# icyveins7/pydsproutines

Hardware: AMD Instinct MI355X
Metric: CAF Msamples/s (4k template x 256 freq bins) (higher is better)
Workload: dtype f32

## Files before the change

### pydsproutines_amd/csrc/caf_fused.hip

```cpp
#include <algorithm>
#include <cstdlib>
#include <type_traits>

#include "caf_internal.h"
#include "caf_fft_dev.h"
#include "caf_wave.h"

namespace caf {

constexpr int FB = 16384;
constexpr int FP_P1 = 4384;
constexpr int FP_IM = 16 * FP_P1;
constexpr int F_LDS_BYTES = 2 * FP_IM;
constexpr int F_LDS_DATA = F_LDS_BYTES / 8;
__host__ __device__ constexpr int fp_row2(int n2) { return ((n2 >> 1) & 3) * 1088 + ((n2 & 1) + 2 * (n2 >> 3)) * 256; }
static_assert(fp_row2(15) + 256 <= FP_P1 && FP_P1 % 256 == 32, "planar image geometry");

#define CAF_AS1 __attribute__((address_space(1)))
#define CAF_AS4 __attribute__((address_space(4)))
typedef float v2f_t __attribute__((ext_vector_type(2)));
typedef float v4f_t __attribute__((ext_vector_type(4)));
typedef int v2i_t __attribute__((ext_vector_type(2)));
__device__ __forceinline__ float2 ld2(const float2* base, uint32_t elem) {
    const uint64_t u = *reinterpret_cast<const CAF_AS1 uint64_t*>((const CAF_AS1 char*)base + (elem << 3));
// ... 398 lines not shown
                bii = up ? pk_i[n4] : bii;
            }
            const uint32_t dloc = pk_d0 + (16u * bii + 64u * bq) * 64u;
            unsigned long long key = bvv < 0.f ? 0ull : (((unsigned long long)__float_as_uint(bvv) << 32) | (uint32_t)~dloc);
            key = wave_max(key);
            if ((tid & 63) == 0) {
                PeakRec r;
                r.v = key ? __uint_as_float((uint32_t)(key >> 32)) : -1.f;
                r.delay = key ? (int32_t)(f1->shift_start + f1_rel0 + (int64_t)(uint32_t)~(uint32_t)key) : 0x7fffffff;
                r.f = 0;
                f1->partial[(int64_t)h * f1->ppt + (int64_t)f1->blk_abs * 16 + (tid >> 6)] = r;
            }
        }
    }
    if (MODE == 2 || MODE == 5) {
        const int n1 = tid & 15, n2 = (tid >> 4) & 15, q = tid >> 8;
#pragma unroll
        for (int i = 0; i < 4; ++i)
#pragma unroll
            for (int n4 = 0; n4 < 4; ++n4) {
                const int tile = 16 * i + 64 * n4 + (n2 >> 2) + 4 * q;
                const int oo = 4 * i + n4;
                if (tile < tiles_per_blk) {
                    const uint32_t off = ((uint32_t)tile * 64u + (uint32_t)(n1 + 16 * (n2 & 3))) << 2;
                    gst1_wt(vt, off, bv[oo]);
                    __hip_atomic_store(reinterpret_cast<CAF_AS1 int32_t*>((CAF_AS1 char*)imax + off),
                                       (int32_t)(h0 + ((bi[oo >> 2] >> (8 * (oo & 3))) & 0xffu)), __ATOMIC_RELAXED,
                                       __HIP_MEMORY_SCOPE_AGENT);
                }
            }
    }
}

template <int N_> struct caf_ic { static constexpr int value = N_; };
template <int MODE, int NVH, bool FOLD, int R, bool PART = false>
__device__ __forceinline__ void fused_item2q(float2* __restrict__ s_d, const float2* __restrict__ s_tw2,
                                             const float2* __restrict__ s_tw3, const float2* __restrict__ xb,
                                             const float2* __restrict__ hc,
                                             const int32_t* __restrict__ shifts, const float2* __restrict__ tw1,
                                             int32_t table_mode, int32_t nfreq, int32_t nhyp, int blk, int h0, int h1,
                                             int32_t tiles_per_blk, float* __restrict__ vt, int32_t npart = 1,
                                             const F1Direct* __restrict__ f1 = nullptr) {
    static_assert(FOLD || R == 0, "the output residue exists in the folded form only");
    static_assert(MODE == 1 || MODE == 4, "|y|^2 tiles (write-through) or complex-QF rows");
    static_assert(!FOLD || NVH == 0, "folded form: only the lower half of each residue's transform holds valid delays");
    static_assert(!PART || FOLD, "partitioned templates ride on the folded form");
    constexpr int ROW = FOLD ? 4 * FB : 2 * FB;
    using pt_t = typename std::conditional<FOLD, float4, float2>::type;
    const int tid = threadIdx.x;
    const lds_char* img = (const lds_char*)s_d;
    const uint32_t img0 = __builtin_amdgcn_readfirstlane((uint32_t)(uintptr_t)img);
    const uint32_t wave_u = __builtin_amdgcn_readfirstlane((uint32_t)tid >> 6);
    const uint32_t m0_x1 = img0 + wave_u * 256u, m0_w = img0 + wave_u * (uint32_t)FP_P1;
    const uint32_t m2 = fp_m2((uint32_t)tid);
    const float2 w = ld2(tw1, 1024u + m2);
    float2 base0 = make_float2(1.f, 0.f);
    if (R) {
        float sn, cs;
        sincospif((float)m2 * (1.0f / 16384.0f), &sn, &cs);
        base0 = make_float2(cs, sn);
    }
    const float* xp = (const float*)(xb + (int64_t)blk * ROW);
    float* vt_blk = vt + (int64_t)blk * tiles_per_blk * nhyp * 64;
    const __amdgpu_buffer_rsrc_t rvt = buf_of(uniform_ptr(vt_blk), (uint32_t)tiles_per_blk * (uint32_t)nhyp * 256u);
    const int n1o = tid & 15, n2o = (tid >> 4) & 15, qo = tid >> 8;
    uint32_t f1_bytes = 0;
    int64_t f1_rel0 = 0;
    __amdgpu_buffer_rsrc_t rie = rvt, f1_r0 = rvt;
    float f1_ts = 0.f;
    if constexpr (MODE == 4) {
        f1_rel0 = (int64_t)f1->blk_abs * f1->step;
        int64_t nv = f1->num_shifts - f1_rel0;
        if (nv > f1->step) nv = f1->step;
        f1_bytes = (uint32_t)nv * 4u;
        rie = buf_of(uniform_ptr(f1->inv_e + f1_rel0), f1_bytes);
    }
    const float* hrow_o;
    uint32_t hb_o;
    const float* hrow_n;
    uint32_t hb_n;
    auto row_of = [&](int h, const float*& hrow, uint32_t& hb) {
        const int rows_per = PART ? npart : 1;
        if (table_mode) {
            hrow = (const float*)(hc + (int64_t)h * rows_per * ROW);
            hb = (uint32_t)tid;
        } else {
            const int t = h / nfreq;
            const int32_t sh = *((const CAF_AS4 int32_t*)shifts + (h - t * nfreq)) >> 1;
            hrow = (const float*)(hc + (int64_t)t * rows_per * ROW);
            hb = fp_hbase(m2, sh);
        }
    };
    auto issue = [&](pt_t* bx, pt_t* bh, const float* hrow, uint32_t hb, auto cc_, auto a0_, auto np_, uint32_t lz) __attribute__((always_inline)) {
        constexpr int CC = decltype(cc_)::value, A0 = decltype(a0_)::value, NP = decltype(np_)::value;
#pragma unroll
        for (int k = 0; k < NP; ++k) {
            const uint32_t a = (uint32_t)(A0 + k);
// ... 460 lines not shown
        float v = -1.f;
        if (lane < nrows) {
            v = s_rowv[lane];
            const int64_t o = (int64_t)t * num_shifts + rel0 + lane;
            if (row_max) row_max[o] = v < 0.f ? __builtin_nanf("") : v;
            if (row_arg) row_arg[o] = s_rowi[lane];
        }
        if (partial) {
            float b = v;
            int32_t bidx = lane;
            wave_argmax(b, bidx);
            if (lane == 0) {
                PeakRec r;
                r.v = b;
                r.delay = (int32_t)(shift_start + rel0 + bidx);
                r.f = s_rowi[bidx];
                partial[(int64_t)t * partial_per_tmpl + pidx] = r;
            }
        }
    }
}


constexpr int PQ_FFT_NEXT = 0, PQ_TR_NEXT = 1, PQ_FFT_XCD = 4, PQ_DONE = 12;
constexpr int PQ_TILES = 16;

__device__ __forceinline__ int32_t pq_load(const int32_t* p) {
    return __hip_atomic_load(p, __ATOMIC_RELAXED, __HIP_MEMORY_SCOPE_AGENT);
}
__device__ __forceinline__ const CAF_AS4 PersistParams* params_of(const PersistParams* p) {
    uint64_t v = reinterpret_cast<uint64_t>(p);
    asm volatile("" : "+s"(v));
    return reinterpret_cast<const CAF_AS4 PersistParams*>(v);
}
typedef float v4f_u_t __attribute__((ext_vector_type(4), aligned(4)));
typedef int v4i_u_t __attribute__((ext_vector_type(4), aligned(4)));

constexpr int TW_H = 32;
constexpr int TW_PITCH = TW_H + 1;
constexpr int TW_LDS = 64 * TW_PITCH;

template <bool SURF, int DS>
__device__ __forceinline__ void transpose_wave(float* __restrict__ lds, const PersistParams* pp, int z, int tile0) {
    const CAF_AS4 PersistParams* P = params_of(pp);
    const int32_t ntmpl = P->ntmpl, nfreq = P->nfreq, step = P->step, tiles_per_blk = P->tiles_per_blk;
    const int64_t num_shifts = P->num_shifts, shift_start = P->shift_start;
    const int wave_id = __builtin_amdgcn_readfirstlane((int)(threadIdx.x >> 6));
    const int lane = threadIdx.x & 63;
    float* s_w = lds + wave_id * TW_LDS;
    const int tile = tile0 + wave_id;
    if (tile >= tiles_per_blk) return;
    const int blk = P->blk0 + z;
    const int sl0 = DS == 2 ? 128 * (tile & 255) + (tile >> 8) : tile * 64;
    const int64_t rel0 = (int64_t)blk * step + sl0;
    int64_t nv = num_shifts - (int64_t)blk * step;
    if (nv > step) nv = step;
    const int nrows = sl0 < nv ? (int)min((int64_t)64, (nv - sl0 + DS - 1) / DS) : 0;
    const int64_t pidx = (int64_t)blk * tiles_per_blk + tile;
    PeakRec* partial = P->partial;
    const int64_t ppt = P->partial_per_tmpl;
    const int s4 = 4 * (lane & 15), fq = lane >> 4;
    const int nsteps = (nfreq + TW_H - 1) / TW_H;
    for (int t = 0; t < ntmpl; ++t) {
        if (nrows == 0) {
            if (lane == 0 && partial) {
                PeakRec r;
// ... 310 lines not shown
        if (wave_id == 0) {
            int32_t* pq = P->pq;
            const int n_fft = P->n_fft, n_tr = P->n_tr, ngroups = P->ngroups;
            int next = -1;
            const int t = __builtin_amdgcn_readfirstlane(pq_load(&pq[PQ_TR_NEXT]));
            if (t < n_tr) {
                const bool fft_left = __builtin_amdgcn_readfirstlane(pq_load(&pq[PQ_FFT_NEXT])) < n_fft;
                if (!fft_left || __builtin_amdgcn_readfirstlane(pq_load(&pq[PQ_DONE + t / ipb])) >= ngroups) {
                    int my = 0;
                    if (lane0) my = atomicAdd(&pq[PQ_TR_NEXT], 1);
                    my = __builtin_amdgcn_readfirstlane(my);
                    if (my < n_tr) {
                        pq_wait_block(pq, my, ipb, ngroups, lane0);
                        next = my;
                    }
                }
            }
            if (lane0) *s_next = next;
        }
        __syncthreads();
        item = __builtin_amdgcn_readfirstlane(*s_next);
        __syncthreads();
        if (item < 0) return;
    }
}

__device__ __forceinline__ void pq_mark(const PersistParams* pp, int slot, int v) {
    int32_t* d = params_of(pp)->dbg;
    if (d) __hip_atomic_store(&d[blockIdx.x * 8 + slot], v, __ATOMIC_RELAXED, __HIP_MEMORY_SCOPE_SYSTEM);
}

typedef __attribute__((address_space(3))) float2 lds_float2;
template <int KIND, int NV4>
__device__ __attribute__((noinline)) void persistent_fft_item(lds_float2* s_d, const lds_float2* s_tw2,
                                                              const lds_float2* s_tw3, const PersistParams* pp_in,
                                                              int item_in) {
    const PersistParams* pp = uniform_ptr(pp_in);
    const int item = __builtin_amdgcn_readfirstlane(item_in);
    const CAF_AS4 PersistParams* P = params_of(pp);
    const int ngroups = P->ngroups, hyp_per_wg = P->hyp_per_wg, nhyp = P->nhyp;
    const int blk = item / ngroups;
    const int grp = item - blk * ngroups;
    int h0 = grp * hyp_per_wg;
    int h1 = min(h0 + hyp_per_wg, nhyp);
    if (const int gpt = P->gpt) {
        const int t = grp / gpt;
        h0 = t * P->nfreq + (grp - t * gpt) * hyp_per_wg;
        h1 = min(h0 + hyp_per_wg, (t + 1) * P->nfreq);
    }
    if (KIND == 3) {
        F1Direct f1;
        f1.out0 = P->cqf;
        f1.out1 = nullptr;
        f1.partial = nullptr;
        f1.ppt = 0;
        f1.shift_start = 0;
        f1.inv_e = P->inv_e;
        f1.tscale = P->tscale;
        f1.num_shifts = P->num_shifts;
        f1.step = P->step;
        f1.blk_abs = P->blk0 + blk;
        fused_item<1024, 4, NV4>((float2*)s_d, (const float2*)s_tw2, (const float2*)s_tw3, P->xb, P->hc, P->shifts, P->tw1,
                                 P->table_mode, P->nfreq, nhyp, blk, h0, h1, P->tiles_per_blk, nullptr, nullptr, &f1);
    } else if (KIND == 2 || KIND == 4) {
        F1Direct f1;
        f1.out0 = P->row_max ? P->row_max : P->surface;
        f1.out1 = (P->row_max && P->surface) ? P->surface : nullptr;
        f1.inv_e = P->inv_e;
        f1.tscale = P->tscale;
        f1.num_shifts = P->num_shifts;
        f1.step = P->step;
        f1.blk_abs = P->blk0 + blk;
        f1.partial = P->partial;
        f1.ppt = P->partial_per_tmpl;
        f1.shift_start = P->shift_start;
        fused_item<1024, 3, NV4, KIND == 4>((float2*)s_d, (const float2*)s_tw2, (const float2*)s_tw3, P->xb, P->hc, P->shifts, P->tw1,
                                            P->table_mode, P->nfreq, nhyp, blk, h0, h1, P->tiles_per_blk, nullptr, nullptr, &f1);
    } else if (KIND == 5) {
        F1Direct f1;
        f1.out0 = P->surface_t;
        f1.out1 = nullptr;
        f1.partial = nullptr;
        f1.ppt = 0;
        f1.shift_start = 0;
        f1.inv_e = P->inv_e;
        f1.tscale = P->tscale;
        f1.num_shifts = P->num_shifts;
        f1.step = P->step;
        f1.blk_abs = P->blk0 + blk;
        const int64_t o = ((int64_t)blk * ngroups + grp) * P->tiles_per_blk * 64;
        fused_item<1024, 5, NV4>((float2*)s_d, (const float2*)s_tw2, (const float2*)s_tw3, P->xb, P->hc, P->shifts, P->tw1,
                                 P->table_mode, P->nfreq, nhyp, blk, h0, h1, P->tiles_per_blk, P->vmax + o, P->imax + o, &f1);
    } else if (KIND == 1) {
        const int64_t o = ((int64_t)blk * ngroups + grp) * P->tiles_per_blk * 64;
        fused_item<1024, 2, NV4>((float2*)s_d, (const float2*)s_tw2, (const float2*)s_tw3, P->xb, P->hc, P->shifts, P->tw1,
                            P->table_mode, P->nfreq, nhyp, blk, h0, h1, P->tiles_per_blk, P->vmax + o, P->imax + o);
    } else {
        fused_item<1024, 1, NV4>((float2*)s_d, (const float2*)s_tw2, (const float2*)s_tw3, P->xb, P->hc, P->shifts, P->tw1,
                            P->table_mode, P->nfreq, nhyp, blk, h0, h1, P->tiles_per_blk, P->vt);
    }
    __builtin_amdgcn_fence(__ATOMIC_RELEASE, "workgroup");
    __syncthreads();
    if (threadIdx.x == 0)
        __hip_atomic_fetch_add(&params_of(pp)->pq[PQ_DONE + blk], 1, __ATOMIC_RELAXED, __HIP_MEMORY_SCOPE_AGENT);
}

__device__ __forceinline__ void cq_params(const CAF_AS4 PersistParams* P, int blk, F1Direct& f1) {
    f1.out0 = P->cqf;
    f1.out1 = nullptr;
    f1.partial = nullptr;
    f1.ppt = 0;
    f1.shift_start = 0;
    f1.inv_e = P->inv_e;
    f1.tscale = P->tscale;
    f1.num_shifts = P->num_shifts;
    f1.step = P->step;
    f1.blk_abs = P->blk0 + blk;
}
template <int NVH, bool CQ>
__device__ __attribute__((noinline)) void persistent_fft_item2(lds_float2* s_d, const lds_float2* s_tw2, const lds_float2* s_tw3,
                                                               const PersistParams* pp_in, int item_in) {
    const PersistParams* pp = uniform_ptr(pp_in);
    const int item = __builtin_amdgcn_readfirstlane(item_in);
    const CAF_AS4 PersistParams* P = params_of(pp);
    const int ngroups = P->ngroups, hyp_per_wg = P->hyp_per_wg, nhyp = P->nhyp;
    const int blk = item / ngroups;
    const int grp = item - blk * ngroups;
    const int h0 = grp * hyp_per_wg;
    const int h1 = min(h0 + hyp_per_wg, nhyp);
    if constexpr (CQ) {
        F1Direct f1;
        cq_params(P, blk, f1);
        fused_item2q<4, NVH, false, 0>((float2*)s_d, (const float2*)s_tw2, (const float2*)s_tw3, P->xb, P->hc, P->shifts, P->tw1,
                                       P->table_mode, P->nfreq, nhyp, blk, h0, h1, P->tiles_per_blk, P->vt, 1, &f1);
    } else
    fused_item2q<1, NVH, false, 0>((float2*)s_d, (const float2*)s_tw2, (const float2*)s_tw3, P->xb, P->hc, P->shifts, P->tw1, P->table_mode,
                                   P->nfreq, nhyp, blk, h0, h1, P->tiles_per_blk, P->vt);
    __builtin_amdgcn_fence(__ATOMIC_RELEASE, "workgroup");
    __syncthreads();
    if (threadIdx.x == 0)
        __hip_atomic_fetch_add(&params_of(pp)->pq[PQ_DONE + blk], 1, __ATOMIC_RELAXED, __HIP_MEMORY_SCOPE_AGENT);
}

template <int R, bool PART, bool CQ>
__device__ __attribute__((noinline)) void persistent_fft_item2f(lds_float2* s_d, const lds_float2* s_tw2, const lds_float2* s_tw3,
                                                                const PersistParams* pp_in, int item_in) {
    const PersistParams* pp = uniform_ptr(pp_in);
    const int item = __builtin_amdgcn_readfirstlane(item_in);
    const CAF_AS4 PersistParams* P = params_of(pp);
    const int ngroups = P->ngroups, hyp_per_wg = P->hyp_per_wg, nhyp = P->nhyp;
    const int blk = item / ngroups;
    const int grp = (item - blk * ngroups) >> 1;
    const int h0 = grp * hyp_per_wg;
    const int h1 = min(h0 + hyp_per_wg, nhyp);
    if constexpr (CQ) {
        F1Direct f1;
        cq_params(P, blk, f1);
        fused_item2q<4, 0, true, R, PART>((float2*)s_d, (const float2*)s_tw2, (const float2*)s_tw3, P->xb, P->hc, P->shifts, P->tw1,
                                          P->table_mode, P->nfreq, nhyp, blk, h0, h1, P->tiles_per_blk, P->vt, PART ? P->npart : 1, &f1);
    } else
    fused_item2q<1, 0, true, R, PART>((float2*)s_d, (const float2*)s_tw2, (const float2*)s_tw3, P->xb, P->hc, P->shifts, P->tw1, P->table_mode,
                                      P->nfreq, nhyp, blk, h0, h1, P->tiles_per_blk, P->vt, PART ? P->npart : 1);
    __builtin_amdgcn_fence(__ATOMIC_RELEASE, "workgroup");
    __syncthreads();
    if (threadIdx.x == 0)
        __hip_atomic_fetch_add(&params_of(pp)->pq[PQ_DONE + blk], 1, __ATOMIC_RELAXED, __HIP_MEMORY_SCOPE_AGENT);
}

template <bool STATS>
__global__ __launch_bounds__(1024) void k_caf_persistent(const PersistParams* __restrict__ pp) {
    static_assert(16 * TW_LDS * 4 <= F_LDS_DATA * 8, "transposer patches must fit the FFT image");
    __shared__ __attribute__((aligned(16))) float2 s_d[F_LDS_DATA];
    __shared__ float2 s_tw2[2 * 16 * 64];
    __shared__ float2 s_tw3[2 * 16 * 4];
    __shared__ int32_t s_cmd[2];
    const int tid = threadIdx.x;
    {
        const CAF_AS4 PersistParams* P = params_of(pp);
        const float2* tw23 = P->tw23;
        s_tw2[tid] = tw23[tid];
        s_tw2[1024 + tid] = tw23[1088 + tid];
        if (tid < 64) {
            s_tw3[tid] = tw23[1024 + tid];
            s_tw3[64 + tid] = tw23[1088 + 1024 + tid];
        }
    }
    __syncthreads();
    const int wave_id = __builtin_amdgcn_readfirstlane(tid >> 6);
    const bool lane0 = (tid & 63) == 0;
    uint64_t tmark = STATS ? wall_clock64() : 0;
    const uint32_t t_start = (uint32_t)tmark;
    uint32_t t_claim = 0, t_fft = 0, t_tile = 0, c_fft = 0, c_tile = 0;
    for (;;) {
        if (wave_id == 0) {
            const CAF_AS4 PersistParams* P = params_of(pp);
            int32_t* pq = P->pq;
            const int n_fft = P->n_fft, n_tr = P->n_tr, ipb = P->ipb, ngroups = P->ngroups;
            const bool prefer_tr = (int)((blockIdx.x >> 3) & 31) >= 32 - P->tr_slots;
            int kind = 0, item = 0, spins = 0;
            for (;;) {
                const bool fft_left = __builtin_amdgcn_readfirstlane(pq_load(&pq[PQ_FFT_NEXT])) < n_fft;
                if (prefer_tr || !fft_left) {
                    const int t = __builtin_amdgcn_readfirstlane(pq_load(&pq[PQ_TR_NEXT]));
                    if (t < n_tr) {
                        if (!fft_left || __builtin_amdgcn_readfirstlane(pq_load(&pq[PQ_DONE + t / ipb])) >= ngroups) {
                            int my = 0;
                            if (lane0) my = atomicAdd(&pq[PQ_TR_NEXT], 1);
                            my = __builtin_amdgcn_readfirstlane(my);
                            if (my < n_tr) {
                                kind = 2;
                                item = my;
                                break;
                            }
                            continue;
                        }
                    } else if (!fft_left) {
                        break;
                    }
                }
                if (fft_left) {
                    const int nblk = P->nblk;
                    const int x0 = (int)(blockIdx.x & 7);
                    int got = -1;
                    if (P->block_log2 < 15) {
                        int i = 0;
// ... 13 lines not shown
                    if (got >= 0) {
                        if (lane0) atomicAdd(&pq[PQ_FFT_NEXT], 1);
                        kind = 1;
                        item = got;
                        break;
                    }
                    continue;
                }
                __builtin_amdgcn_s_sleep(64);
                if (++spins > (1 << 22)) break;
            }
            if (kind == 2) pq_wait_block(pq, item, ipb, ngroups, lane0);
            if (lane0) {
                s_cmd[0] = kind;
                s_cmd[1] = item;
            }
            if (STATS) {
                const uint64_t now = wall_clock64();
                t_claim += (uint32_t)(now - tmark);
                tmark = now;
            }
        }
        __syncthreads();
        const int kind = __builtin_amdgcn_readfirstlane(s_cmd[0]), item = __builtin_amdgcn_readfirstlane(s_cmd[1]);
        if (kind == 0) {
            if (STATS && tid == 0) {
                pq_mark(pp, 0, (int)t_claim);
                pq_mark(pp, 1, (int)t_fft);
                pq_mark(pp, 2, (int)t_tile);
                pq_mark(pp, 3, (int)c_fft);
                pq_mark(pp, 4, (int)c_tile);
                pq_mark(pp, 5, (int)t_start);
                pq_mark(pp, 6, (int)(uint32_t)wall_clock64());
            }
            break;
        }
        if (kind == 1) {
            if (__builtin_amdgcn_readfirstlane(params_of(pp)->block_log2) == 16) {
                const bool odd_r = ((item - (item / params_of(pp)->ngroups) * params_of(pp)->ngroups) & 1) != 0;
                const bool part = __builtin_amdgcn_readfirstlane(params_of(pp)->npart) > 1, cq = params_of(pp)->cqf != nullptr;
#define CAF_FFT_ROLE2F(RR, PP, CC) persistent_fft_item2f<RR, PP, CC>((lds_float2*)s_d, (const lds_float2*)s_tw2, (const lds_float2*)s_tw3, pp, item)
                if (cq) {
                    if (part) { if (odd_r) CAF_FFT_ROLE2F(1, true, true); else CAF_FFT_ROLE2F(0, true, true); }
                    else { if (odd_r) CAF_FFT_ROLE2F(1, false, true); else CAF_FFT_ROLE2F(0, false, true); }
                } else if (part) {
                    if (odd_r) CAF_FFT_ROLE2F(1, true, false); else CAF_FFT_ROLE2F(0, true, false);
                } else {
                    if (odd_r) CAF_FFT_ROLE2F(1, false, false); else CAF_FFT_ROLE2F(0, false, false);
                }
#undef CAF_FFT_ROLE2F
            } else if (__builtin_amdgcn_readfirstlane(params_of(pp)->block_log2) == 15) {
                const int tpb2 = __builtin_amdgcn_readfirstlane(params_of(pp)->tiles_per_blk);
                const bool cq = params_of(pp)->cqf != nullptr;
#define CAF_FFT_ROLE2(NN, CC) persistent_fft_item2<NN, CC>((lds_float2*)s_d, (const lds_float2*)s_tw2, (const lds_float2*)s_tw3, pp, item)
                if (tpb2 <= 256) { if (cq) CAF_FFT_ROLE2(0, true); else CAF_FFT_ROLE2(0, false); }
                else if (tpb2 <= 384) { if (cq) CAF_FFT_ROLE2(2, true); else CAF_FFT_ROLE2(2, false); }
                else { if (cq) CAF_FFT_ROLE2(4, true); else CAF_FFT_ROLE2(4, false); }
#undef CAF_FFT_ROLE2
            }
            else {
                const int kind3 = params_of(pp)->cqf ? 3
                                  : params_of(pp)->surface_t ? 5
                                  : __builtin_amdgcn_readfirstlane(params_of(pp)->f1_direct) ? (params_of(pp)->partial ? 4 : 2)
                                  : __builtin_amdgcn_readfirstlane(params_of(pp)->nosurf) ? 1 : 0;
                const int tpb = __builtin_amdgcn_readfirstlane(params_of(pp)->tiles_per_blk);
#define CAF_FFT_ROLE(K, Q) persistent_fft_item<K, Q>((lds_float2*)s_d, (const lds_float2*)s_tw2, (const lds_float2*)s_tw3, pp, item)
                if (tpb <= 128) {
                    if (kind3 == 5) CAF_FFT_ROLE(5, 2); else if (kind3 == 4) CAF_FFT_ROLE(4, 2); else if (kind3 == 3) CAF_FFT_ROLE(3, 2); else if (kind3 == 2) CAF_FFT_ROLE(2, 2); else if (kind3 == 1) CAF_FFT_ROLE(1, 2); else CAF_FFT_ROLE(0, 2);
                } else if (tpb <= 192) {
                    if (kind3 == 5) CAF_FFT_ROLE(5, 3); else if (kind3 == 4) CAF_FFT_ROLE(4, 3); else if (kind3 == 3) CAF_FFT_ROLE(3, 3); else if (kind3 == 2) CAF_FFT_ROLE(2, 3); else if (kind3 == 1) CAF_FFT_ROLE(1, 3); else CAF_FFT_ROLE(0, 3);
                } else {
                    if (kind3 == 5) CAF_FFT_ROLE(5, 4); else if (kind3 == 4) CAF_FFT_ROLE(4, 4); else if (kind3 == 3) CAF_FFT_ROLE(3, 4); else if (kind3 == 2) CAF_FFT_ROLE(2, 4); else if (kind3 == 1) CAF_FFT_ROLE(1, 4); else CAF_FFT_ROLE(0, 4);
                }
#undef CAF_FFT_ROLE
            }
            if (STATS) {
                const uint64_t now = wall_clock64();
                t_fft += (uint32_t)(now - tmark);
                tmark = now;
                ++c_fft;
            }
        } else {
            persistent_tile_run((lds_float*)s_d, (lds_int*)&s_cmd[1], pp, item);
            if (STATS) {
                const uint64_t now = wall_clock64();
                t_tile += (uint32_t)(now - tmark);
                tmark = now;
                ++c_tile;
            }
        }
    }
}

__global__ void k_persist_setup(PersistParams h, PersistParams* d) {
    int32_t* pq = h.pq;
    const int n = PQ_DONE + h.nblk;
    for (int i = threadIdx.x; i < n; i += blockDim.x) pq[i] = 0;
    if (threadIdx.x == 0) *d = h;
}

void launch_caf_persistent(const PersistParams* h, PersistParams* d_params, int32_t n_wgs, hipStream_t st) {
    hipLaunchKernelGGL(k_persist_setup, dim3(1), dim3(256), 0, st, *h, d_params);
    const dim3 grid((unsigned)n_wgs), block(1024);
    const PersistParams* dp = d_params;
    if (h->dbg)
        hipLaunchKernelGGL((k_caf_persistent<true>), grid, block, 0, st, dp);
    else
        hipLaunchKernelGGL((k_caf_persistent<false>), grid, block, 0, st, dp);
}

void launch_fused_caf(const float2* xb, const float2* hc, const int32_t* shifts, const float2* tw1,
                      const float2* tw23, int32_t table_mode, int32_t nfreq, int32_t nhyp, int32_t hyp_per_wg,
                      int32_t nblk, int32_t tiles_per_blk, float* vt, hipStream_t st) {
// ... 39 lines not shown
```

### pydsproutines_amd/csrc/caf_internal.h

```cpp
#pragma once
#include <hip/hip_runtime.h>
#include <stdint.h>

#include "caf.h"
#include "caf_energy.h"

#include <map>
#include <mutex>
#include <string>
#include <utility>
#include <vector>

namespace caf {

constexpr int MUL_THREADS = 256;
constexpr int MAG_THREADS = 256;
constexpr int MAG_S = 64;
constexpr int MAG_F = 128;

inline int64_t energy_prefix_doubles(int64_t m) { return ((m + 2) & ~(int64_t)1) + (m + 63) / 64 + 1; }

struct PeakRec {
    float v;
    int32_t delay;
// ... 199 lines not shown
void launch_parity_major(const float2* in, float2* out, int64_t rows, int32_t half, hipStream_t st, bool butterfly = false);
void launch_parity_pairs(const float2* in, float2* out, int64_t rows, int32_t quarter, hipStream_t st);
void launch_fused_caf(const float2* xb, const float2* hc, const int32_t* shifts, const float2* tw1,
                      const float2* tw23, int32_t table_mode, int32_t nfreq, int32_t nhyp, int32_t hyp_per_wg,
                      int32_t nblk, int32_t tiles_per_blk, float* vt, hipStream_t st);
void launch_transpose_norm_argmax(const float* vt, int32_t ntmpl, int32_t nfreq, const float* tscale,
                                  const float* inv_e, int64_t num_shifts, int64_t shift_start, int32_t step,
                                  int32_t blk0, int32_t nblk, int32_t tiles_per_blk, float* surface, float* row_max,
                                  int32_t* row_arg, PeakRec* partial, int64_t partial_per_tmpl, hipStream_t st);

struct PersistParams {
    const float2* xb;
    const float2* hc;
    const int32_t* shifts;
    const float2* tw1;
    const float2* tw23;
    float* vt;
    int32_t table_mode, nfreq, nhyp, hyp_per_wg, nblk, tiles_per_blk;
    int32_t block_log2;
    int32_t dstride;
    int32_t npart;
    int32_t ntmpl, step, blk0;
    int32_t gpt;
    const float* tscale;
    const float* inv_e;
    int64_t num_shifts, shift_start;
    float* surface;
    float* row_max;
    int32_t* row_arg;
    PeakRec* partial;
    int64_t partial_per_tmpl;
    int32_t* pq;
    int32_t tr_slots, ngroups, n_fft, ipb, n_tr;
    int32_t nosurf;
    int32_t f1_direct;
    float* cqf;
    float* surface_t;
    float* vmax;
    int32_t* imax;
    int32_t* dbg;
};
void launch_butterfly_order(const float2* in, float2* out, int64_t nchunks, hipStream_t st);
void launch_caf_persistent(const PersistParams* h, PersistParams* d_params, int32_t n_wgs, hipStream_t st);

struct FftPlan {
    void* plan = nullptr;
    void* info = nullptr;
    void* work = nullptr;
    size_t work_bytes = 0;
    int exec(void* in, void* out, hipStream_t st);
    void* slot = nullptr;
    hipEvent_t last_use = nullptr;
    bool last_use_pending = false;

private:
    friend int fft_plan_acquire(FftPlan*, bool, size_t, size_t, size_t, bool);
    friend void fft_plan_release(FftPlan*, hipStream_t);
    int create(bool inverse, size_t len, size_t batch, size_t dist, bool inplace);
    void destroy();
};
int fft_plan_acquire(FftPlan* out, bool inverse, size_t len, size_t batch, size_t dist, bool inplace = true);
void fft_plan_release(FftPlan* p, hipStream_t st = nullptr);
int fft_rows(const float2* in, float2* out, int64_t rows, int64_t len, bool inverse, hipStream_t st);

#define CAF_REQUIRE(cond, msg)      \
    do {                            \
// ... 8 lines not shown
```

### pydsproutines_amd/csrc/caf_plan.hip

```cpp
#include <algorithm>
#include <cmath>
#include <complex>
#include <cstring>
#include <mutex>
#include <vector>

#include <unistd.h>

#include "caf_internal.h"

namespace caf {

static thread_local std::string g_last_error;
void set_error(const std::string& msg) { g_last_error = msg; }

}

using namespace caf;

static int env_int(const char* name, int dflt, bool* is_set = nullptr) {
    const char* e = getenv(name);
    if (is_set) *is_set = e != nullptr;
    return e ? atoi(e) : dflt;
}
// ... 896 lines not shown
static PersistParams fill_persist_params(const caf_plan_t* p, const PersistMode& m, int64_t b0, int32_t nbk, const Call& c) {
    PersistParams h;
    std::memset(&h, 0, sizeof(h));
    h.xb = (p->B >= 32768 ? p->d_xb2 : p->d_xb) + b0 * (int64_t)p->B;
    h.hc = p->d_hc;
    h.shifts = p->d_shifts;
    h.tw1 = p->d_tw1;
    h.tw23 = p->d_tw23;
    h.vt = p->d_vt;
    h.table_mode = p->mul_mode == 2 ? 1 : 0;
    h.nfreq = p->F;
    h.nhyp = p->T * p->F;
    h.hyp_per_wg = m.hyp_per_wg;
    h.nblk = nbk;
    h.tiles_per_blk = p->tiles_per_blk;
    h.block_log2 = p->B == 65536 ? 16 : p->B == 32768 ? 15 : 14;
    h.dstride = p->B == 65536 ? 2 : 1;
    h.npart = p->npart;
    h.ntmpl = p->T;
    h.step = p->step;
    h.blk0 = (int32_t)b0;
    h.gpt = m.gpt;
    h.tscale = p->d_tscale;
    h.inv_e = p->d_inv_e;
    h.num_shifts = c.num_shifts;
    h.shift_start = c.shift_start;
    h.surface = c.d_surface;
    h.row_max = c.d_row_max;
    h.row_arg = c.d_row_arg;
    h.partial = c.want_peak && (!m.f1_direct || m.f1_item_peaks) ? p->d_partial : nullptr;
    h.partial_per_tmpl = p->partial_per_tmpl;
    h.pq = p->d_pq;
    h.tr_slots = p->tr_slots;
    h.ngroups = m.ngroups;
    h.n_fft = nbk * m.ngroups;
    h.ipb = (p->tiles_per_blk + 15) / 16;
    h.n_tr = m.f1_direct || m.cqf_rows ? 0 : nbk * h.ipb;
    h.nosurf = m.nosurf;
    h.f1_direct = m.f1_direct ? 1 : 0;
    h.cqf = c.d_cqf;
    h.surface_t = c.d_surface_t;
    h.vmax = p->d_vt;
    h.imax = reinterpret_cast<int32_t*>(p->d_vt + m.imax_off);
    return h;
}

static void persist_report(caf_plan p, const PersistParams& h, const int32_t* h_dbg, bool surface, hipStream_t st) {
    hipEvent_t ev;
    (void)hipEventCreate(&ev);
    (void)hipEventRecord(ev, st);
    bool done = false;
    for (int i = 0; i < 80 && !done; ++i) {
        done = hipEventQuery(ev) == hipSuccess;
        if (!done) usleep(100000);
    }
    if (!done) {
        fprintf(stderr, "[caf persistent] kernel still running after 8 s: aborting the process\n");
        _exit(3);
    }
    std::vector<int32_t> q(4 + h.nblk);
    (void)hipMemcpy(q.data(), p->d_pq, q.size() * 4, hipMemcpyDeviceToHost);
    double sum[2][5] = {{0}};
    int cnt[2] = {0, 0};
    uint32_t t0 = 0xffffffffu, t1 = 0, tl = 0;
    for (int w = 0; w < p->n_cus; ++w) {
        const int pref = ((w >> 3) & 31) >= 32 - p->tr_slots;
        ++cnt[pref];
        for (int k = 0; k < 5; ++k) sum[pref][k] += h_dbg[8 * w + k];
        t0 = std::min(t0, (uint32_t)h_dbg[8 * w + 5]);
        tl = std::max(tl, (uint32_t)h_dbg[8 * w + 5]);
        t1 = std::max(t1, (uint32_t)h_dbg[8 * w + 6]);
    }
    fprintf(stderr, "[caf persistent] n_fft=%d n_tr=%d | fft_next=%d tr_next=%d watchdog=%d,%d | first start -> last end "
            "%.0f us, last start +%.0f us\n", h.n_fft, h.n_tr, q[0], q[1], q[2], q[3], (t1 - t0) / 100.0, (tl - t0) / 100.0);
    for (int r = 0; r < 2; ++r)
        if (cnt[r])
            fprintf(stderr,
                    "  %s workgroups (%d): claim+wait %.0f us, fft %.0f us in %.1f items (%.1f us each), tiles %.0f us "
                    "in %.1f items (%.1f us each)\n",
                    r ? "tile-first" : "fft-first", cnt[r], sum[r][0] / cnt[r] / 100.0, sum[r][1] / cnt[r] / 100.0,
                    sum[r][3] / cnt[r], sum[r][3] > 0 ? sum[r][1] / sum[r][3] / 100.0 : 0.0,
                    sum[r][2] / cnt[r] / 100.0, sum[r][4] / cnt[r],
                    sum[r][4] > 0 ? sum[r][2] / sum[r][4] / 100.0 : 0.0);
    const char* lst = getenv("CAF_PERSIST_TILE_ONLY");
    if (!lst) return;
    PersistParams h2 = h;
    h2.n_fft = 0;
    h2.ngroups = 0;
    h2.dbg = nullptr;
    hipEvent_t e0, e1;
    (void)hipEventCreate(&e0);
    (void)hipEventCreate(&e1);
    for (const char* s = lst; *s;) {
        const int k = atoi(s);
        while (*s && *s != ',') ++s;
        if (*s == ',') ++s;
        if (k < 1) continue;
        (void)hipEventRecord(e0, st);
        launch_caf_persistent(&h2, p->d_params, k, st);
        (void)hipEventRecord(e1, st);
        (void)hipEventSynchronize(e1);
        float ms = 0.f;
        (void)hipEventElapsedTime(&ms, e0, e1);
        const double bytes = (double)h2.n_tr * 16.0 * 64.0 * p->F * 4.0 * (surface ? 2.0 : 1.0);
        fprintf(stderr, "  tile role alone on %3d workgroups: %.2f ms, %.1f us per item, %.1f GB/s per CU, %.2f TB/s\n",
                k, ms, ms * 1e3 * k / h2.n_tr, bytes / (ms * 1e-3) / k / 1e9, bytes / (ms * 1e-3) / 1e12);
    }
}

static int32_t poison_tiles(caf_plan p, hipStream_t st) {
    CAF_HIP_TRY(hipMemsetD32Async((hipDeviceptr_t)p->d_vt, (int)POISON_VT, (size_t)vt_floats(p, p->nb, (int64_t)p->T * p->F), st));
    return CAF_OK;
}

// ... 170 lines not shown
```

Baseline: 1273.

## Chain persistent FFT items to prefetch next block across item boundaries

Adds a chained variant of the fused FFT item in which, on the last hypothesis of an item, wave 0 claims the next work item from the persistent queue and the kernel prefetches the next block's input and template rows into registers while the current transform finishes. Completion of the previous block is published late, after its stores drain, so the next item starts without returning to the scheduler loop. The goal is to hide item-boundary overhead (claim, sync, first-row global loads) in the persistent kernel. It is enabled by default through an env flag but only for FFT-preferring workgroups, and it adds code complexity, extra register pressure and changed ordering of done counters.

After: 1283, median of 6. No clear change (+0.8%).

```diff
diff --git a/pydsproutines_amd/csrc/caf_fused.hip b/pydsproutines_amd/csrc/caf_fused.hip
--- a/pydsproutines_amd/csrc/caf_fused.hip
+++ b/pydsproutines_amd/csrc/caf_fused.hip
@@ -454,6 +454,210 @@
     }
 }
 
+struct ChainCtx {
+    const PersistParams* pp;
+    __attribute__((address_space(3))) int32_t* s_nxt;
+    int32_t ngroups, hyp_per_wg;
+    int32_t claims;
+    int32_t items;
+};
+__device__ __forceinline__ int chain_claim(const PersistParams* pp, bool lane0);
+__device__ __forceinline__ void publish_wait();
+__device__ __forceinline__ void chain_publish(const PersistParams* pp, int blk);
+
+template <int NV4>
+__device__ __forceinline__ int fused_item_chain(float2* __restrict__ s_d, const float2* __restrict__ s_tw2,
+                                                const float2* __restrict__ s_tw3, const float2* __restrict__ xb,
+                                                const float2* __restrict__ hc, const int32_t* __restrict__ shifts,
+                                                const float2* __restrict__ tw1, int32_t table_mode, int32_t nfreq,
+                                                int32_t nhyp, int blk, int h0, int h1, int32_t tiles_per_blk,
+                                                float* __restrict__ vt, ChainCtx* ch) {
+    const int tid = threadIdx.x;
+    const lds_char* img = (const lds_char*)s_d;
+    const uint32_t img0 = __builtin_amdgcn_readfirstlane((uint32_t)(uintptr_t)img);
+    const uint32_t wave_u = __builtin_amdgcn_readfirstlane((uint32_t)tid >> 6);
+    const uint32_t m0_x1 = img0 + wave_u * 256u, m0_w = img0 + wave_u * (uint32_t)FP_P1;
+    const uint32_t m2 = fp_m2((uint32_t)tid);
+    constexpr int nv4 = NV4;
+    const float2 w = ld2(tw1, 1024u + m2);
+    __amdgpu_buffer_rsrc_t rvt = buf_of(uniform_ptr(vt + (int64_t)blk * tiles_per_blk * nhyp * 64),
+                                        (uint32_t)tiles_per_blk * (uint32_t)nhyp * 256u);
+    const float2* hrow_cur;
+    uint32_t hb_cur;
+    auto row_of = [&](int h) {
+        if (table_mode) {
+            hrow_cur = hc + (int64_t)h * FB;
+            hb_cur = (uint32_t)tid;
+        } else {
+            const int t = h / nfreq;
+            const int32_t sh = *((const CAF_AS4 int32_t*)shifts + (h - t * nfreq));
+            hrow_cur = hc + (int64_t)t * FB;
+            hb_cur = fp_hbase(m2, sh);
+        }
+    };
+    float2 pr[16], xr[16];
+    {
+        const float2* xp = xb + (int64_t)blk * FB;
+#pragma unroll
+        for (int a = 0; a < 16; ++a) xr[a] = ld2(xp, 1024u * a + m2);
+    }
+    row_of(h0);
+#pragma unroll
+    for (int a = 0; a < 16; ++a) pr[a] = cmul(xr[a], ld2(hrow_cur, (1024u * a + hb_cur) & (FB - 1)));
+
+    int h = h0;
+    int pend_blk = -1;
+    auto hyp = [&](auto edge_c) __attribute__((always_inline)) -> int {
+        constexpr bool EDGE = decltype(edge_c)::value;
+        const bool last = EDGE && h + 1 >= h1;
+        uint32_t hoff = (uint32_t)h * 256u;
+        asm volatile("" : "+s"(hoff));
+        int lz = 0;
+        asm volatile("" : "+v"(lz));
+        if (EDGE) {
+            if (last && wave_u == 0) {
+                const int got = ch->claims ? chain_claim(ch->pp, (tid & 63) == 0) : -1;
+                if ((tid & 63) == 0) *ch->s_nxt = got;
+            }
+        }
+        float2 v1[16];
+#pragma unroll
+        for (int a = 0; a < 16; ++a) {
+            float px = pr[a].x, py = pr[a].y;
+            asm volatile("" : "+v"(px), "+v"(py));
+            v1[a] = make_float2(px, py);
+        }
+        idft16(v1);
+        {
+            float2 p = w;
+            asm volatile("" : "+v"(p.x), "+v"(p.y));
+            const float2 wj = p;
+            v1[1] = cmul(v1[1], p);
+#pragma unroll
+            for (int n1 = 2; n1 < 16; ++n1) {
+                p = cmul(p, wj);
+                v1[n1] = cmul(v1[n1], p);
+            }
+        }
+        if (EDGE) {
+            if (pend_blk >= 0) publish_wait();
+        }
+        __syncthreads();
+        if (EDGE) {
+            if (pend_blk >= 0) {
+                if (tid == 0) chain_publish(ch->pp, pend_blk);
+                pend_blk = -1;
+            }
+        }
+        lds_rows16c<FP_P1>(m0_x1, v1);
+        __syncthreads();
+        int n_blk = -1, n_h0 = 0, n_h1 = 0;
+        if (EDGE) {
+            if (last) {
+                const int it = __builtin_amdgcn_readfirstlane(*ch->s_nxt);
+                if (it >= 0) {
+                    n_blk = it / ch->ngroups;
+                    n_h0 = (it - n_blk * ch->ngroups) * ch->hyp_per_wg;
+                    n_h1 = min(n_h0 + ch->hyp_per_wg, nhyp);
+                }
+            }
+        }
+        if (EDGE && n_blk >= 0) {
+            const float2* xn = xb + (int64_t)n_blk * FB;
+#pragma unroll
+            for (int a = 0; a < 16; ++a) xr[a] = ld2(xn, 1024u * a + m2);
+            row_of(n_h0);
+        } else
+            row_of(last ? h : h + 1);
+        constexpr int HP2 = 5;
+        float2 hn[16];
+#pragma unroll
+        for (int a = 0; a < HP2; ++a) hn[a] = ld2(hrow_cur, ((1024u * a + hb_cur) & (FB - 1)) + lz);
+        {
+            float2 v[16];
+            const uint32_t rd2 = fp_rd2((uint32_t)(tid + lz)), rd2i = fp_im(rd2);
+            const lds_tw_ptr t2 = tw_base(s_tw2, fp_cd2((uint32_t)(tid + lz)));
+#pragma unroll
+            for (int bh = 0; bh < 4; ++bh) lds_get4c(img, rd2 + 256u * bh, rd2i + 256u * bh, v[4 * bh], v[4 * bh + 1], v[4 * bh + 2], v[4 * bh + 3]);
+            idft16(v);
+#pragma unroll
+            for (int n2 = 1; n2 < 16; ++n2) v[n2] = cmul(v[n2], tw_ld(t2, n2 * 64));
+            lds_rows16c_x2(m0_w, v);
+        }
+        __builtin_amdgcn_wave_barrier();
+#pragma unroll
+        for (int a = HP2; a < 16; ++a) hn[a] = ld2(hrow_cur, (1024u * a + hb_cur) & (FB - 1));
+        {
+            float2 v[16];
+            const uint32_t rd3 = fp_rd3((uint32_t)(tid + lz)), rd3i = fp_im(rd3);
+#pragma unroll
+            for (int ch4 = 0; ch4 < 4; ++ch4) lds_get4c(img, rd3 + 64u * ch4, rd3i + 64u * ch4, v[4 * ch4], v[4 * ch4 + 1], v[4 * ch4 + 2], v[4 * ch4 + 3]);
+            idft16(v);
+            const lds_tw_ptr t3 = tw_base(s_tw3, (uint32_t)((tid & 3) + lz));
+#pragma unroll
+            for (int n3 = 1; n3 < 16; ++n3) v[n3] = cmul(v[n3], tw_ld(t3, n3 * 4));
+            lds_rows16c<256>(m0_w, v);
+        }
+        __syncthreads();
+        {
+            const int n1 = tid & 15, n2 = (tid >> 4) & 15, q = tid >> 8;
+            const uint32_t rd4 = fp_rd4((uint32_t)tid), rd4i = fp_im(rd4);
+            __builtin_amdgcn_sched_barrier(0);
+            float2 pf0, pf1, pf2, pf3;
+            lds_get4c(img, rd4, rd4i, pf0, pf1, pf2, pf3);
+            __builtin_amdgcn_sched_barrier(0);
+#pragma unroll
+            for (int a = 0; a < 16; ++a) pr[a] = cmul(xr[a], hn[a]);
+            __builtin_amdgcn_sched_barrier(0);
+#pragma unroll
+            for (int i = 0; i < 4; ++i) {
+                uint32_t lzi = 0;
+                asm volatile("" : "+v"(lzi));
+                float2 a0, a1, a2, a3;
+                if (i == 0)
+                    a0 = pf0, a1 = pf1, a2 = pf2, a3 = pf3;
+                else
+                    lds_get4c(img, rd4 + 1024u * i + lzi, rd4i + 1024u * i + lzi, a0, a1, a2, a3);
+                const float2 s02 = cadd(a0, a2), d02 = csub(a0, a2), s13 = cadd(a1, a3), d13 = mulj(csub(a1, a3));
+#pragma unroll
+                for (int n4 = 0; n4 < 4; ++n4) {
+                    if (n4 >= nv4) continue;
+                    const float2 yq = n4 == 0 ? cadd(s02, s13) : n4 == 1 ? cadd(d02, d13) : n4 == 2 ? csub(s02, s13) : csub(d02, d13);
+                    const int tile_u = 16 * i + 64 * n4;
+                    const int tile_t = (n2 >> 2) + 4 * q;
+                    const uint32_t soff = (uint32_t)tile_u * (uint32_t)nhyp * 256u + hoff;
+                    const uint32_t voff = ((uint32_t)tile_t * (uint32_t)nhyp * 64u + (uint32_t)(n1 + 16 * (n2 & 3))) << 2;
+                    const float val = __builtin_fmaf(yq.x, yq.x, yq.y * yq.y);
+                    tile_store<1>(rvt, voff, soff, val);
+                }
+                __builtin_amdgcn_sched_barrier(0);
+            }
+            __builtin_amdgcn_sched_barrier(0);
+        }
+        if (EDGE) {
+            if (last) {
+                if (n_blk < 0) return 2;
+                pend_blk = blk;
+                blk = n_blk;
+                h0 = n_h0;
+                h1 = n_h1;
+                h = n_h0;
+                rvt = buf_of(uniform_ptr(vt + (int64_t)blk * tiles_per_blk * nhyp * 64), (uint32_t)tiles_per_blk * (uint32_t)nhyp * 256u);
+                ++ch->items;
+                return 1;
+            }
+        }
+        return 0;
+    };
+    for (;;) {
+        const int r = hyp(std::true_type{});
+        if (r == 2) break;
+        if (r == 1) continue;
+        for (++h; h + 1 < h1; ++h) hyp(std::false_type{});
+    }
+    return blk;
+}
+
 template <int N_> struct caf_ic { static constexpr int value = N_; };
 template <int MODE, int NVH, bool FOLD, int R, bool PART = false>
 __device__ __forceinline__ void fused_item2q(float2* __restrict__ s_d, const float2* __restrict__ s_tw2,
@@ -484,7 +688,7 @@
     }
     const float* xp = (const float*)(xb + (int64_t)blk * ROW);
     float* vt_blk = vt + (int64_t)blk * tiles_per_blk * nhyp * 64;
-    const __amdgpu_buffer_rsrc_t rvt = buf_of(uniform_ptr(vt_blk), (uint32_t)tiles_per_blk * (uint32_t)nhyp * 256u);
+    __amdgpu_buffer_rsrc_t rvt = buf_of(uniform_ptr(vt_blk), (uint32_t)tiles_per_blk * (uint32_t)nhyp * 256u);
     const int n1o = tid & 15, n2o = (tid >> 4) & 15, qo = tid >> 8;
     uint32_t f1_bytes = 0;
     int64_t f1_rel0 = 0;
@@ -1011,6 +1215,22 @@
     uint64_t v = reinterpret_cast<uint64_t>(p);
     asm volatile("" : "+s"(v));
     return reinterpret_cast<const CAF_AS4 PersistParams*>(v);
+}
+__device__ __forceinline__ int chain_claim(const PersistParams* pp, bool lane0) {
+    const CAF_AS4 PersistParams* P = params_of(pp);
+    int i = 0;
+    if (lane0) i = atomicAdd(&P->pq[PQ_FFT_XCD], 1);
+    i = __builtin_amdgcn_readfirstlane(i);
+    if (i >= P->n_fft) return -1;
+    if (lane0) atomicAdd(&P->pq[PQ_FFT_NEXT], 1);
+    return i;
+}
+__device__ __forceinline__ void publish_wait() {
+    asm volatile("s_waitcnt vmcnt(0)" ::: "memory");
+    __builtin_amdgcn_fence(__ATOMIC_RELEASE, "workgroup");
+}
+__device__ __forceinline__ void chain_publish(const PersistParams* pp, int blk) {
+    __hip_atomic_fetch_add(&params_of(pp)->pq[PQ_DONE + blk], 1, __ATOMIC_RELAXED, __HIP_MEMORY_SCOPE_AGENT);
 }
 typedef float v4f_u_t __attribute__((ext_vector_type(4), aligned(4)));
 typedef int v4i_u_t __attribute__((ext_vector_type(4), aligned(4)));
@@ -1387,14 +1607,15 @@
 
 typedef __attribute__((address_space(3))) float2 lds_float2;
 template <int KIND, int NV4>
-__device__ __attribute__((noinline)) void persistent_fft_item(lds_float2* s_d, const lds_float2* s_tw2,
-                                                              const lds_float2* s_tw3, const PersistParams* pp_in,
-                                                              int item_in) {
+__device__ __attribute__((noinline)) int persistent_fft_item(lds_float2* s_d, const lds_float2* s_tw2,
+                                                             const lds_float2* s_tw3, const PersistParams* pp_in,
+                                                             int item_in, lds_int* s_nxt) {
     const PersistParams* pp = uniform_ptr(pp_in);
     const int item = __builtin_amdgcn_readfirstlane(item_in);
     const CAF_AS4 PersistParams* P = params_of(pp);
     const int ngroups = P->ngroups, hyp_per_wg = P->hyp_per_wg, nhyp = P->nhyp;
-    const int blk = item / ngroups;
+    int blk = item / ngroups;
+    int nitems = 1;
     const int grp = item - blk * ngroups;
     int h0 = grp * hyp_per_wg;
     int h1 = min(h0 + hyp_per_wg, nhyp);
@@ -1451,13 +1672,22 @@
         fused_item<1024, 2, NV4>((float2*)s_d, (const float2*)s_tw2, (const float2*)s_tw3, P->xb, P->hc, P->shifts, P->tw1,
                             P->table_mode, P->nfreq, nhyp, blk, h0, h1, P->tiles_per_blk, P->vmax + o, P->imax + o);
     } else {
-        fused_item<1024, 1, NV4>((float2*)s_d, (const float2*)s_tw2, (const float2*)s_tw3, P->xb, P->hc, P->shifts, P->tw1,
-                            P->table_mode, P->nfreq, nhyp, blk, h0, h1, P->tiles_per_blk, P->vt);
-    }
-    __builtin_amdgcn_fence(__ATOMIC_RELEASE, "workgroup");
+        ChainCtx ch;
+        ch.pp = pp;
+        ch.s_nxt = s_nxt;
+        ch.ngroups = ngroups;
+        ch.hyp_per_wg = hyp_per_wg;
+        ch.claims = (int)((blockIdx.x >> 3) & 31) < 32 - P->tr_slots && P->gpt == 0 && __builtin_amdgcn_readfirstlane(P->chain) != 0;
+        ch.items = 1;
+        blk = fused_item_chain<NV4>((float2*)s_d, (const float2*)s_tw2, (const float2*)s_tw3, P->xb, P->hc, P->shifts, P->tw1,
+                                    P->table_mode, P->nfreq, nhyp, blk, h0, h1, P->tiles_per_blk, P->vt, &ch);
+        nitems = ch.items;
+    }
+    publish_wait();
     __syncthreads();
     if (threadIdx.x == 0)
         __hip_atomic_fetch_add(&params_of(pp)->pq[PQ_DONE + blk], 1, __ATOMIC_RELAXED, __HIP_MEMORY_SCOPE_AGENT);
+    return nitems;
 }
 
 __device__ __forceinline__ void cq_params(const CAF_AS4 PersistParams* P, int blk, F1Direct& f1) {
@@ -1491,7 +1721,7 @@
     } else
     fused_item2q<1, NVH, false, 0>((float2*)s_d, (const float2*)s_tw2, (const float2*)s_tw3, P->xb, P->hc, P->shifts, P->tw1, P->table_mode,
                                    P->nfreq, nhyp, blk, h0, h1, P->tiles_per_blk, P->vt);
-    __builtin_amdgcn_fence(__ATOMIC_RELEASE, "workgroup");
+    publish_wait();
     __syncthreads();
     if (threadIdx.x == 0)
         __hip_atomic_fetch_add(&params_of(pp)->pq[PQ_DONE + blk], 1, __ATOMIC_RELAXED, __HIP_MEMORY_SCOPE_AGENT);
@@ -1516,7 +1746,7 @@
     } else
     fused_item2q<1, 0, true, R, PART>((float2*)s_d, (const float2*)s_tw2, (const float2*)s_tw3, P->xb, P->hc, P->shifts, P->tw1, P->table_mode,
                                       P->nfreq, nhyp, blk, h0, h1, P->tiles_per_blk, P->vt, PART ? P->npart : 1);
-    __builtin_amdgcn_fence(__ATOMIC_RELEASE, "workgroup");
+    publish_wait();
     __syncthreads();
     if (threadIdx.x == 0)
         __hip_atomic_fetch_add(&params_of(pp)->pq[PQ_DONE + blk], 1, __ATOMIC_RELAXED, __HIP_MEMORY_SCOPE_AGENT);
@@ -1529,6 +1759,7 @@
     __shared__ float2 s_tw2[2 * 16 * 64];
     __shared__ float2 s_tw3[2 * 16 * 4];
     __shared__ int32_t s_cmd[2];
+    __shared__ int32_t s_nxt;
     const int tid = threadIdx.x;
     {
         const CAF_AS4 PersistParams* P = params_of(pp);
@@ -1545,7 +1776,7 @@
     const bool lane0 = (tid & 63) == 0;
     uint64_t tmark = STATS ? wall_clock64() : 0;
     const uint32_t t_start = (uint32_t)tmark;
-    uint32_t t_claim = 0, t_fft = 0, t_tile = 0, c_fft = 0, c_tile = 0;
+    uint32_t t_claim = 0, t_fft = 0, t_tile = 0, c_fft = 0, c_tile = 0, c_call = 0;
     for (;;) {
         if (wave_id == 0) {
             const CAF_AS4 PersistParams* P = params_of(pp);
@@ -1625,10 +1856,12 @@
                 pq_mark(pp, 4, (int)c_tile);
                 pq_mark(pp, 5, (int)t_start);
                 pq_mark(pp, 6, (int)(uint32_t)wall_clock64());
+                pq_mark(pp, 7, (int)c_call);
             }
             break;
         }
         if (kind == 1) {
+            int n_run = 1;
             if (__builtin_amdgcn_readfirstlane(params_of(pp)->block_log2) == 16) {
                 const bool odd_r = ((item - (item / params_of(pp)->ngroups) * params_of(pp)->ngroups) & 1) != 0;
                 const bool part = __builtin_amdgcn_readfirstlane(params_of(pp)->npart) > 1, cq = params_of(pp)->cqf != nullptr;
@@ -1657,7 +1890,7 @@
                                   : __builtin_amdgcn_readfirstlane(params_of(pp)->f1_direct) ? (params_of(pp)->partial ? 4 : 2)
                                   : __builtin_amdgcn_readfirstlane(params_of(pp)->nosurf) ? 1 : 0;
                 const int tpb = __builtin_amdgcn_readfirstlane(params_of(pp)->tiles_per_blk);
-#define CAF_FFT_ROLE(K, Q) persistent_fft_item<K, Q>((lds_float2*)s_d, (const lds_float2*)s_tw2, (const lds_float2*)s_tw3, pp, item)
+#define CAF_FFT_ROLE(K, Q) n_run = persistent_fft_item<K, Q>((lds_float2*)s_d, (const lds_float2*)s_tw2, (const lds_float2*)s_tw3, pp, item, (lds_int*)&s_nxt)
                 if (tpb <= 128) {
                     if (kind3 == 5) CAF_FFT_ROLE(5, 2); else if (kind3 == 4) CAF_FFT_ROLE(4, 2); else if (kind3 == 3) CAF_FFT_ROLE(3, 2); else if (kind3 == 2) CAF_FFT_ROLE(2, 2); else if (kind3 == 1) CAF_FFT_ROLE(1, 2); else CAF_FFT_ROLE(0, 2);
                 } else if (tpb <= 192) {
@@ -1671,7 +1904,8 @@
                 const uint64_t now = wall_clock64();
                 t_fft += (uint32_t)(now - tmark);
                 tmark = now;
-                ++c_fft;
+                c_fft += (uint32_t)__builtin_amdgcn_readfirstlane(n_run);
+                ++c_call;
             }
         } else {
             persistent_tile_run((lds_float*)s_d, (lds_int*)&s_cmd[1], pp, item);
diff --git a/pydsproutines_amd/csrc/caf_internal.h b/pydsproutines_amd/csrc/caf_internal.h
--- a/pydsproutines_amd/csrc/caf_internal.h
+++ b/pydsproutines_amd/csrc/caf_internal.h
@@ -255,6 +255,7 @@
     int64_t partial_per_tmpl;
     int32_t* pq;
     int32_t tr_slots, ngroups, n_fft, ipb, n_tr;
+    int32_t chain;
     int32_t nosurf;
     int32_t f1_direct;
     float* cqf;
diff --git a/pydsproutines_amd/csrc/caf_plan.hip b/pydsproutines_amd/csrc/caf_plan.hip
--- a/pydsproutines_amd/csrc/caf_plan.hip
+++ b/pydsproutines_amd/csrc/caf_plan.hip
@@ -952,6 +952,7 @@
     h.partial_per_tmpl = p->partial_per_tmpl;
     h.pq = p->d_pq;
     h.tr_slots = p->tr_slots;
+    h.chain = env_int("CAF_PERSIST_CHAIN", 1) != 0;
     h.ngroups = m.ngroups;
     h.n_fft = nbk * m.ngroups;
     h.ipb = (p->tiles_per_blk + 15) / 16;
@@ -980,13 +981,14 @@
     }
     std::vector<int32_t> q(4 + h.nblk);
     (void)hipMemcpy(q.data(), p->d_pq, q.size() * 4, hipMemcpyDeviceToHost);
-    double sum[2][5] = {{0}};
+    double sum[2][5] = {{0}}, calls[2] = {0, 0};
     int cnt[2] = {0, 0};
     uint32_t t0 = 0xffffffffu, t1 = 0, tl = 0;
     for (int w = 0; w < p->n_cus; ++w) {
         const int pref = ((w >> 3) & 31) >= 32 - p->tr_slots;
         ++cnt[pref];
         for (int k = 0; k < 5; ++k) sum[pref][k] += h_dbg[8 * w + k];
+        calls[pref] += h_dbg[8 * w + 7];
         t0 = std::min(t0, (uint32_t)h_dbg[8 * w + 5]);
         tl = std::max(tl, (uint32_t)h_dbg[8 * w + 5]);
         t1 = std::max(t1, (uint32_t)h_dbg[8 * w + 6]);
@@ -996,10 +998,10 @@
     for (int r = 0; r < 2; ++r)
         if (cnt[r])
             fprintf(stderr,
-                    "  %s workgroups (%d): claim+wait %.0f us, fft %.0f us in %.1f items (%.1f us each), tiles %.0f us "
+                    "  %s workgroups (%d): claim+wait %.0f us, fft %.0f us in %.1f items (%.1f us each; %.1f calls), tiles %.0f us "
                     "in %.1f items (%.1f us each)\n",
                     r ? "tile-first" : "fft-first", cnt[r], sum[r][0] / cnt[r] / 100.0, sum[r][1] / cnt[r] / 100.0,
-                    sum[r][3] / cnt[r], sum[r][3] > 0 ? sum[r][1] / sum[r][3] / 100.0 : 0.0,
+                    sum[r][3] / cnt[r], sum[r][3] > 0 ? sum[r][1] / sum[r][3] / 100.0 : 0.0, calls[r] / cnt[r],
                     sum[r][2] / cnt[r] / 100.0, sum[r][4] / cnt[r],
                     sum[r][4] > 0 ? sum[r][2] / sum[r][4] / 100.0 : 0.0);
     const char* lst = getenv("CAF_PERSIST_TILE_ONLY");
```
